# CSB5/lofreq

Hardware: AMD Instinct MI355X
Metric: pileup columns/sec at depth 10000 (higher is better)
Workload: dtype f64

## Files before the change

### lofreq_amd/csrc/lfq_api.hip

```cpp
#include "lfq_bound.h"
#include "lfq_ctx.h"

namespace {

struct LfqDeviceStreams {
    hipStream_t stream = nullptr, dps = nullptr, side[2] = {nullptr, nullptr};
    hipEvent_t ev_tail[3] = {nullptr, nullptr, nullptr};
    bool tail_recorded = false;
    hipEvent_t ev_end = nullptr;
    bool end_recorded = false;
    int refs = 0;
};
std::mutex g_streams_m;
LfqDeviceStreams g_streams[64];

bool acquire_streams(int device, lfq_ctx *c);
void release_streams(int device);

void *pin_acquire_impl(lfq_ctx *c, size_t bytes, int *slot)
{
    int best = -1, empty = -1, smallest = -1;
    for (int i = 0; i < LFQ_PIN_SLOTS; i++) {
        auto &b = c->pin_pool[i];
        if (b.used) {
// ... 231 lines not shown
    for (;;) {
        {
            std::unique_lock<std::mutex> lk(*c->lm);
            c->lcv->wait(lk, [&] { return c->leader_go > 0 || c->leader_stop; });
            if (c->leader_stop) {
                return;
            }
            c->leader_go--;
        }
        int64_t n = 0;
        if (hipEventSynchronize(c->ev_heavy) == hipSuccess) {
            n = std::min<int64_t>(std::max<int64_t>(*(volatile int32_t *)c->h_nheavy, 0), c->heavy_cap);
        }
        lfq_sb_precompute(c->h_tuples, 3 * n);
        {
            std::lock_guard<std::mutex> lk(*c->lm);
            c->sb_pending--;
        }
        c->lcv->notify_all();
    }
}

int ensure_workspace(lfq_ctx *c, int64_t ncols)
{
    if (ncols > c->ws_cols) {
        int64_t cap = 0;
        int64_t want = ncols + ncols / 8 + 1024;
        if (c->d_flags) (void)hipFree(c->d_flags);
        if (c->d_prefix) (void)hipFree(c->d_prefix);
        if (c->d_entries) (void)hipFree(c->d_entries);
        if (c->d_tiles) (void)hipFree(c->d_tiles);
        if (c->d_unsplit) (void)hipFree(c->d_unsplit);
        if (c->d_retry) (void)hipFree(c->d_retry);
        c->d_unsplit = nullptr;
        c->d_retry = nullptr;
        c->d_flags = nullptr;
        c->d_prefix = nullptr;
        c->d_entries = nullptr;
        c->d_tiles = nullptr;
        c->ws_cols = 0;
        LFQ_TRY(grow(&c->d_flags, &cap, want));
        cap = 0;
        LFQ_TRY(grow(&c->d_prefix, &cap, want));
        cap = 0;
        LFQ_TRY(grow(&c->d_entries, &cap, want));
        cap = 0;
        LFQ_TRY(grow(&c->d_tiles, &cap, 2 * (want / 1024 + 8 * (LFQ_MAX_SEGMENTS + 1))));
        cap = 0;
        LFQ_TRY(grow(&c->d_unsplit, &cap, want));
        cap = 0;
        LFQ_TRY(grow(&c->d_retry, &cap, want));
        c->ws_cols = want;
    }
    return LFQ_OK;
}


}

void *lfq_pin_acquire(lfq_ctx *c, size_t bytes, int *slot) { return pin_acquire_impl(c, bytes, slot); }

extern "C" {

void *lfq_host_alloc(size_t bytes)
{
    void *p = nullptr;
    if (hipHostMalloc(&p, bytes ? bytes : 1, hipHostMallocDefault) != hipSuccess) {
        (void)hipGetLastError();
        return nullptr;
    }
    return p;
}

void lfq_host_free(void *p)
{
    if (p) {
        (void)hipHostFree(p);
    }
}
int lfq_create(lfq_ctx **out, int device_ordinal)
{
    if (!out) {
        return LFQ_ERR_INVALID;
    }
// ... 108 lines not shown
        if (c->h_pin2) (void)hipHostFree(c->h_pin2);
        if (c->d_detlim) (void)hipFree(c->d_detlim);
        if (c->d_sites_in) (void)hipFree(c->d_sites_in);
        if (c->d_sites_out) (void)hipFree(c->d_sites_out);
        for (int i = 0; i < 4; i++) {
            if (c->ev_sites_t[i]) (void)hipEventDestroy(c->ev_sites_t[i]);
        }
        if (c->d_sum) (void)hipFree(c->d_sum);
        if (c->h_sum) (void)hipHostFree(c->h_sum);
        delete c->plp_sum;
        if (c->ev_sum_t[0]) (void)hipEventDestroy(c->ev_sum_t[0]);
        if (c->ev_sum_t[1]) (void)hipEventDestroy(c->ev_sum_t[1]);
        if (c->ev_baq_t[0]) (void)hipEventDestroy(c->ev_baq_t[0]);
        if (c->ev_baq_t[1]) (void)hipEventDestroy(c->ev_baq_t[1]);
        if (c->ev_idq_t[0]) (void)hipEventDestroy(c->ev_idq_t[0]);
        if (c->ev_idq_t[1]) (void)hipEventDestroy(c->ev_idq_t[1]);
        if (c->d_baq_scr) (void)hipFree(c->d_baq_scr);
        if (c->d_baq_expect) (void)hipFree(c->d_baq_expect);
        if (c->d_baq_tmp8) (void)hipFree(c->d_baq_tmp8);
        if (c->d_baq_nflag) (void)hipFree(c->d_baq_nflag);
        if (c->d_baq_itab) (void)hipFree(c->d_baq_itab);
        if (c->d_baq_terms) (void)hipFree(c->d_baq_terms);
        lfq_viterbi_release(c);
        if (c->h_tuples) (void)hipHostFree(c->h_tuples);
        if (c->h_nheavy) (void)hipHostFree(c->h_nheavy);
        if (c->ev_heavy) (void)hipEventDestroy(c->ev_heavy);
    }
    if (!c) {
        return;
    }
    (void)hipSetDevice(c->device);
    if (c->stream) (void)hipStreamSynchronize(c->stream);
    void *bufs[] = {c->d_luts, c->d_flags, c->d_prefix, c->d_entries, c->d_counters, c->d_tiles, c->d_longs, c->d_pool, c->d_unsplit, c->d_retry,
                    c->d_scratch, c->d_counts, c->d_pvals, c->d_stage, c->d_approx_mu};
    for (void *b : bufs) {
        if (b) (void)hipFree(b);
    }
    if (c->h_counters) (void)hipHostFree(c->h_counters);
    for (int i = 0; i < 4; i++) {
        if (c->ev[i]) (void)hipEventDestroy(c->ev[i]);
    }
    for (int i = 0; i < 3; i++) {
        if (c->ev_join[i]) (void)hipEventDestroy(c->ev_join[i]);
        if (i == 0 && c->ev_segw) (void)hipEventDestroy(c->ev_segw);
        if (i == 0 && c->ev_prep) (void)hipEventDestroy(c->ev_prep);
        if (i == 0 && c->ev_mid) (void)hipEventDestroy(c->ev_mid);
    }
    for (int s = 0; s < LFQ_MAX_SEGMENTS; s++) {
        hipEvent_t evs[] = {c->ev_cnt[s][0], c->ev_cnt[s][1], c->ev_scan[s], c->ev_light[s][0], c->ev_light[s][1],
                            c->ev_side[0][s][0], c->ev_side[0][s][1], c->ev_side[1][s][0], c->ev_side[1][s][1]};
        for (hipEvent_t e : evs) {
            if (e) (void)hipEventDestroy(e);
        }
    }
    if (c->own_streams) {
        release_streams(c->device);
    }
    free(c);
}

int lfq_synchronize(lfq_ctx *c)
{
    if (!c) {
        return LFQ_ERR_INVALID;
    }
    LFQ_TRY_HIP(hipStreamSynchronize(c->stream));
    LFQ_TRY_HIP(hipEventSynchronize(c->ev[3]));
// ... 77 lines not shown
    }
    c->cur_col_bytes = 8 + 1 + (T.coverage_plp ? 4 : 0) + (T.num_bases ? 4 : 0) + (P.detlim_af ? 4 : 0);
    LFQ_TRY(lfq_order_after_batch(c, st));
    LFQ_TRY(tail_wait(c, st));
    LFQ_TRY_HIP(hipMemsetAsync(c->d_counters, 0, (LFQ_MAX_SEGMENTS + 1) * LFQ_NCOUNTERS * sizeof(int32_t), st));
    if (ncols > 0) {
        LFQ_TRY_HIP(hipMemsetAsync(c->d_retry, 0, (size_t)ncols, st));
    }
    LFQ_TRY_HIP(hipEventRecord(c->ev[0], st));
    if (ncols == 0) {
        LFQ_TRY_HIP(hipMemcpyAsync(c->h_counters, c->d_counters,
                                   (LFQ_MAX_SEGMENTS + 1) * LFQ_NCOUNTERS * sizeof(int32_t), hipMemcpyDeviceToHost, st));
        LFQ_TRY_HIP(hipEventRecord(c->ev[3], st));
        c->batch_recorded = 1;
        return LFQ_OK;
    }

    int64_t max_depth = tr->max_col_obs;
    if (max_depth <= 0) {
        LFQ_TRY(lfq_launch_maxdepth(T, gcounters, st));
        LFQ_TRY_HIP(hipMemcpyAsync(c->h_counters, gcounters, LFQ_NCOUNTERS * sizeof(int32_t), hipMemcpyDeviceToHost, st));
        LFQ_TRY_HIP(hipStreamSynchronize(st));
        max_depth = c->h_counters[LFQ_GC_MAXDEPTH];
    }
    {
        static const LfqLuts h_luts = [] {
            LfqLuts h;
            fill_luts(&h);
            return h;
        }();
        const bool lb = !P.general && P.def_alt_bq == 0 && P.def_alt_jp < 0.0;
        P.bound_p_lo = (lb && !indel_mode && kn.bound_gate && lfq_count_is_lean(T, P, max_depth))
                           ? lfq_bound_p_lo(h_luts.bq, P.min_alt_bq4, LFQ_BOUND_QLO) : 0.0;
    }
    const int64_t per_block = 3 * max_depth + 72;
    int n_big_blocks = c->n_cu;
    const int64_t budget = (int64_t)1 << 29;
    if (per_block * n_big_blocks > budget) {
        n_big_blocks = (int)std::max<int64_t>(8, budget / per_block);
    }
    LFQ_TRY(grow(&c->d_scratch, &c->scratch_doubles, per_block * n_big_blocks));
    if (!c->d_longs) {
        c->long_cap = 1 << 16;
        c->pool_cells = kn.split_pool_cells;
        LFQ_TRY_HIP(hipMalloc((void **)&c->d_longs, (size_t)c->long_cap * sizeof(LfqLong)));
        LFQ_TRY_HIP(hipMalloc((void **)&c->d_pool, (size_t)std::max(c->pool_cells, 1) * sizeof(LfqSegCell)));
        LFQ_TRY_HIP(hipEventCreateWithFlags(&c->ev_segw, hipEventDisableTiming));
        LFQ_TRY_HIP(hipEventCreateWithFlags(&c->ev_prep, hipEventDisableTiming));
        LFQ_TRY_HIP(hipEventCreateWithFlags(&c->ev_mid, hipEventDisableTiming));
    }

    const int n_seg = 1;
    c->cur_segments = n_seg;
    LFQ_TRY_HIP(hipEventRecord(c->ev_join[2], st));
    LFQ_TRY_HIP(hipStreamWaitEvent(dps, c->ev_join[2], 0));

    bool big_joined = false;
    for (int s = 0; s < n_seg; s++) {
        const int64_t c0 = ncols * s / n_seg, c1 = ncols * (s + 1) / n_seg;
        LfqWork W;
        W.tested_prefix = c->d_prefix;
        W.entries = c->d_entries + c0;
        W.counters = c->d_counters + s * LFQ_NCOUNTERS;
        W.gcounters = gcounters;
        W.block_sums = (int32_t *)(c->d_tiles + 2 * (c0 / 1024 + 8 * s));
        W.long_cap = c->long_cap / n_seg;
        W.pool_cells = c->pool_cells / n_seg;
        W.longs = c->d_longs + (int64_t)s * W.long_cap;
        W.pool = c->d_pool + (int64_t)s * W.pool_cells;
        W.unsplit = c->d_unsplit + c0;

        LFQ_TRY_HIP(hipEventRecord(c->ev_cnt[s][0], st));
        const bool ungated = c->batch_gate == LFQ_GATE_NONE && st == c->stream && !c->priv_stream_on && !single_stream;
        LFQ_TRY(lfq_launch_count(T, c0, c1, P, c->d_luts, d_counts, c->d_flags, max_depth, st, ungated));
        c->cur_sparse_counts = P.sparse_counts && lfq_count_is_shallow(T, P, max_depth);
        LFQ_TRY_HIP(hipEventRecord(c->ev_cnt[s][1], st));

        LFQ_TRY_HIP(hipStreamWaitEvent(dps, c->ev_cnt[s][1], 0));
        LFQ_TRY(lfq_launch_scan(T, c0, c1, c->d_flags, d_counts, W, dps));
        if (P.approx_n > 0) {
            LFQ_TRY(grow(&c->d_approx_mu, &c->approx_mu_bytes, (c1 - c0) * 8));
            LFQ_TRY(lfq_launch_approx_gate(T, P, c->d_luts, d_counts, W, c1 - c0, (double *)c->d_approx_mu, c->d_flags, dps));
            LFQ_TRY(lfq_launch_scan(T, c0, c1, c->d_flags, d_counts, W, dps, true));
        }
        LFQ_TRY_HIP(hipEventRecord(c->ev_scan[s], dps));
        const bool sb_heavy = n_seg == 1 && !indel_mode && c->leader && !kn.no_sb_precompute;
        auto launch_heavy = [&]() -> int {
            if (P.lazy_strand) {
                LFQ_TRY(lfq_launch_strand_heavy(T, W, d_counts, c->d_tuples_mapped, c->d_nheavy_mapped, c->heavy_cap, 16, dps));
            } else {
                LFQ_TRY(lfq_launch_gather_heavy(W, d_counts, c->d_tuples_mapped, c->d_nheavy_mapped, c->heavy_cap, 16, dps));
            }
            LFQ_TRY_HIP(hipEventRecord(c->ev_heavy, dps));
            {
                std::lock_guard<std::mutex> lk(*c->lm);
                c->leader_go++;
                c->sb_pending++;
            }
            c->lcv->notify_all();
            return LFQ_OK;
        };
        const bool screen = !kn.skip_light && kn.light_kernel != 2;
        if (sb_heavy && !screen) {
            LFQ_TRY(launch_heavy());
        }
        const int64_t seg_cols = c1 - c0;
        const int screen_auto = (c->batch_gate == LFQ_GATE_NONE && !indel_mode) ? (tr->max_col_obs >= 4096 ? 1 : 2) : 4;
        const int light_waves_per_cu = kn.light_kernel == 0 ? screen_auto : 10;
        const int n_light_waves = (int)std::min<int64_t>((int64_t)c->n_cu * light_waves_per_cu, std::max<int64_t>(seg_cols / 8, 4));
        const int n_mid_waves = (int)std::min<int64_t>((int64_t)c->n_cu * 4, std::max<int64_t>(seg_cols, 4));
        const bool run_big = !kn.skip_big, run_mid = !kn.skip_mid;
        const bool dbg_sync = kn.debug_sync != 0;
// ... 832 lines not shown
```

### lofreq_amd/csrc/lfq_ctx.h

```cpp
#ifndef LFQ_CTX_H
#define LFQ_CTX_H

#include <hip/hip_runtime.h>

#include <ctype.h>
#include <float.h>
#include <math.h>
#include <stdio.h>
#include <stdlib.h>
#include <string.h>

#include <algorithm>
#include <chrono>
#include <condition_variable>
#include <mutex>
#include <string>
#include <atomic>
#include <functional>
#include <unistd.h>
#include <fcntl.h>
#include <sys/file.h>
#include <thread>
#include <vector>

// ... 210 lines not shown
    std::vector<char> key_chars;
};

#define LFQ_PIN_SLOTS 40

struct lfq_ctx {
    int device;
    hipStream_t stream;
    LfqLuts *d_luts;
    int64_t ws_cols;
    uint8_t *d_flags;
    uint8_t *d_approx_mu;
    int64_t approx_mu_bytes;
    int32_t *d_prefix, *d_counters;
    LfqEntry *d_entries;
    hipStream_t dps;
    hipStream_t side[2];
    hipEvent_t ev_mid;
    hipEvent_t ev_cnt[LFQ_MAX_SEGMENTS][2];
    hipEvent_t ev_scan[LFQ_MAX_SEGMENTS];
    hipEvent_t ev_light[LFQ_MAX_SEGMENTS][2];
    hipEvent_t ev_side[2][LFQ_MAX_SEGMENTS][2];
    hipEvent_t ev_join[3];
    int cur_segments;
    uint64_t *d_tiles;
    double *d_scratch;
    int64_t scratch_doubles;
    LfqLong *d_longs;
    LfqSegCell *d_pool;
    int32_t long_cap, pool_cells;
    hipEvent_t ev_segw, ev_prep;
    int32_t *d_unsplit;
    uint8_t *d_retry;
    int32_t *h_counters;
    lfq_col_counts *d_counts;
    int64_t counts_cap;
    lfq_col_pvals *d_pvals;
    int64_t pvals_cap;
    uint8_t *d_stage;
    int64_t stage_bytes;
    hipStream_t cur_stream;
    int64_t cur_pvals_cap;
    int64_t cur_ncols;
    hipEvent_t ev[4];
    lfq_kernel_times times;
    lfq_dp_work work;
    int64_t cur_count_read, cur_count_written;
    const uint64_t *cur_col_off;
    int cur_obs_bytes_x2, cur_col_bytes;
    int cur_sparse_counts;
    int n_cu;
    int32_t *h_tuples, *d_tuples_mapped;
    int32_t *h_nheavy, *d_nheavy_mapped;
    int heavy_cap;
    hipEvent_t ev_heavy;
    uint8_t *d_plp_in, *d_plp_out;
    int64_t plp_in_bytes, plp_out_bytes;
    uint8_t *d_tmp[5];
    struct { void *p; size_t cap; } rs_cache[7];
    int priv_stream_on;
    hipStream_t priv_stream;
    hipStream_t up_stream;
    hipEvent_t ev_up;
    hipEvent_t ev_apply;
    uint8_t *h_pin;
    int64_t pin_bytes;
// ... 145 lines not shown
```

### lofreq_amd/csrc/lfq_dp.hip

```cpp
#include <atomic>

#include "lfq_bound.h"
#include "lfq_device.h"

#define LFQ_LN2_HI 6.93147180369123816490e-01
#define LFQ_LN2_LO 1.90821492927058770002e-10
#define LFQ_EXP_UNDERFLOW_X (-708.3964185322641)
#define LFQ_DBL_EPS 2.220446049250313e-16

#ifndef LFQ_HEAVY_WAVES
#define LFQ_HEAVY_WAVES 8
#endif
#ifndef LFQ_DP512_WAVES
#define LFQ_DP512_WAVES 2
#endif

struct LfqColCtx {
    int col;
    uint64_t off0;
    int64_t n_obs;
    int ref_code;
    int median_ref_bq;
    int K;
    int64_t bonf;
// ... 914 lines not shown
            pf.raw = nullptr;
            pf.entry = nullptr;
            lfq_wave_column<1, true, false>(cx, raw, T, P, &s_luts, rows, counts, W, pvals, pvals_capacity, pf);
        }
    }
}


template <int KREG>
__device__ __forceinline__ void lfq_screen_row(double (&v)[KREG], double p, double q)
{
    v[KREG - 1] = fma(v[KREG - 2], p, v[KREG - 1]);
#pragma unroll
    for (int j = KREG - 2; j >= 1; j--) {
        v[j] = fma(v[j - 1], p, v[j] * q);
    }
    v[0] = v[0] * q;
}

#define LFQ_SCREEN_BYTE(w4, j) \
    (((((j) >> 2) == 0 ? (w4).x : ((j) >> 2) == 1 ? (w4).y : ((j) >> 2) == 2 ? (w4).z : (w4).w) >> (8 * ((j) & 3))) & 0xffu)

#define LFQ_SCREEN_CLAIM 128

template <int KREG, bool LB, bool GATE>
__global__ __launch_bounds__(256) void lfq_dp_screen_kernel(LfqTracksDev T, LfqParams P,
                                                            const LfqLuts *__restrict__ g_luts, LfqWork W,
                                                            uint8_t *__restrict__ retry, int max_rounds)
{
    constexpr int MAXK = KREG - 1;
    static_assert(MAXK <= LFQ_BOUND_MAXK, "the bound gate's table");
    static_assert(LB || !GATE, "the bound needs the LB conditions");
    __shared__ LfqLuts s_luts;
    __shared__ LfqBoundTab s_bound;
    lfq_luts_to_lds(&s_luts, g_luts);
    if constexpr (GATE) {
        if (threadIdx.x < LFQ_BOUND_CODES) {
            s_bound.qm[threadIdx.x] = lfq_bound_qm(P.bound_p_lo, threadIdx.x);
        } else if (threadIdx.x >= 64 && threadIdx.x < 64 + LFQ_BOUND_NRK) {
            s_bound.rk[threadIdx.x - 64] = lfq_bound_rk(P.bound_p_lo, (int)threadIdx.x - 64);
        }
    }
    __syncthreads();
    const int lane = lfq_lane();
    const int n_work = W.counters[LFQ_CNT_LIGHT];
    const LfqEntry *list = W.entries;
    const double sig_s = P.sig * (1.0 + P.prune_slack);
    const LfqEvalMasks EM = lfq_eval_masks(P);
    const int xcd0 = (int)(blockIdx.x & 7u);
    int xcd_try = 0;
    int q_next = 0, q_end = 0;

    bool active = false;
    uint64_t off0 = 0;
    int n_obs = 0, rel = 0, K = 0, ref_code = 0, med = 0, rounds = 0, list_idx = 0, n_kept = 0;
    double bonf_d = 1.0;
    double v[KREG];
#pragma unroll
    for (int j = 0; j < KREG; j++) {
        v[j] = 0.0;
    }
    unsigned long long acc_cells = 0, acc_rows = 0;
    int n_retry = 0;

    for (;;) {
        uint64_t need = __ballot(!active);
        while (need != 0ull && (q_next < q_end || xcd_try < 8)) {
            if (q_next >= q_end) {
                const int x = (xcd0 + xcd_try) & 7;
                const int lo = (int)((int64_t)n_work * x / 8), hi = (int)((int64_t)n_work * (x + 1) / 8);
                int32_t *head = &W.counters[LFQ_CNT_XHEAD + 32 * x];
                int b = __hip_atomic_load(head, __ATOMIC_RELAXED, __HIP_MEMORY_SCOPE_AGENT);
                if (b < hi - lo) {
                    b = lfq_claim(head, LFQ_SCREEN_CLAIM);
                }
                if (b >= hi - lo) {
                    xcd_try++;
                    continue;
                }
                q_next = lo + b;
                q_end = min(lo + b + LFQ_SCREEN_CLAIM, hi);
            }
            const int idx = q_next + __popcll(need & ((1ull << lane) - 1ull));
            q_next = min(q_next + __popcll(need), q_end);
            if (!active && idx < q_end) {
                const uint4 *ep = reinterpret_cast<const uint4 *>(list + idx);
                const uint4 a = ep[0], b = ep[1];
                K = (int)b.y;
                if (K > MAXK) {
                    retry[idx] = 1;
                    n_retry++;
                } else {
                    int64_t bonf = P.bonf_base;
                    if (P.bonf_dynamic) {
                        bonf = ((P.bonf_reset_first && P.bonf_base == 1) ? 0 : P.bonf_base)
                               + (int64_t)P.bonf_step * (int)b.x;
                    }
                    bonf_d = (double)bonf;
                    active = true;
                    if constexpr (GATE) {
                        active = !(b.w != 0u && lfq_bound_tail(&s_bound, b.w & (LFQ_BOUND_CODES - 1u), K) * bonf_d > sig_s);
                    }
                    off0 = ((uint64_t)a.y << 32) | a.x;
                    n_obs = (int)a.z;
                    med = (int)(int16_t)(b.z & 0xffffu);
                    ref_code = (int)((b.z >> 16) & 0xffu);
                    rel = -(int)(off0 & 15u);
                    rounds = 0;
                    n_kept = 0;
                    list_idx = idx;
#pragma unroll
                    for (int j = 0; j < KREG; j++) {
                        v[j] = (j == MAXK - K) ? 1.0 : 0.0;
                    }
                }
            }
            need = __ballot(!active);
        }
        if (__ballot(active) == 0ull) {
            break;
        }

        uint4 bqw = make_uint4(0, 0, 0, 0), baqw = make_uint4(~0u, ~0u, ~0u, ~0u), mqw = make_uint4(0, 0, 0, 0);
        uint4 sqw = make_uint4(~0u, ~0u, ~0u, ~0u), ntw = make_uint4(0, 0, 0, 0);
        if (active) {
            const uint64_t wbase = (uint64_t)((int64_t)off0 + rel);
            bqw = *reinterpret_cast<const uint4 *>(T.bq + wbase);
            mqw = *reinterpret_cast<const uint4 *>(T.mq + wbase);
            if (!LB && T.baq) {
                baqw = *reinterpret_cast<const uint4 *>(T.baq + wbase);
            }
            if (!LB && T.sq) {
                sqw = *reinterpret_cast<const uint4 *>(T.sq + wbase);
            }
            if (T.nt_packed) {
// ... 1518 lines not shown
    }
    {
        static std::atomic<unsigned long long> allowed{0ull};
        int dev = 0;
        if (hipGetDevice(&dev) != hipSuccess) {
            return LFQ_ERR_HIP;
        }
        const unsigned long long bit = 1ull << (dev & 63);
        if (!(allowed.load(std::memory_order_acquire) & bit)) {
            const int bytes = (int)sizeof(LfqCombShared);
            if (hipFuncSetAttribute(reinterpret_cast<const void *>(&lfq_dp_combine_kernel<0>),
                                    hipFuncAttributeMaxDynamicSharedMemorySize, bytes) != hipSuccess ||
                hipFuncSetAttribute(reinterpret_cast<const void *>(&lfq_dp_combine_kernel<1>),
                                    hipFuncAttributeMaxDynamicSharedMemorySize, bytes) != hipSuccess) {
                return LFQ_ERR_HIP;
            }
            allowed.fetch_or(bit, std::memory_order_release);
        }
    }
    if (mode == 0) {
        hipLaunchKernelGGL(lfq_dp_fold_kernel<0>, dim3((unsigned)n_blocks * 4), dim3(64 * LFQ_FOLD_WAVES), 0,
                           (hipStream_t)stream, p, d_counts, w, d_pvals, pvals_capacity);
        hipLaunchKernelGGL(lfq_dp_combine_kernel<0>, dim3((unsigned)n_blocks), dim3(LFQ_COMB_THREADS), sizeof(LfqCombShared),
                           (hipStream_t)stream, p, d_counts, w, d_pvals, pvals_capacity, 1);
    } else {
        hipLaunchKernelGGL(lfq_dp_fold_kernel<1>, dim3((unsigned)n_blocks), dim3(64 * LFQ_FOLD_WAVES), 0,
                           (hipStream_t)stream, p, d_counts, w, d_pvals, pvals_capacity);
        hipLaunchKernelGGL(lfq_dp_combine_kernel<1>, dim3((unsigned)n_blocks), dim3(LFQ_COMB_THREADS), sizeof(LfqCombShared),
                           (hipStream_t)stream, p, d_counts, w, d_pvals, pvals_capacity, 1);
    }
    return hipGetLastError() == hipSuccess ? LFQ_OK : LFQ_ERR_HIP;
}

int lfq_launch_dp_quad(const LfqTracksDev &t, const LfqParams &p, const LfqLuts *d_luts,
                       const lfq_col_counts *d_counts, const LfqWork &w, uint8_t *d_retry, lfq_col_pvals *d_pvals,
                       int64_t pvals_capacity, int n_waves, int kreg_hint, void *stream, int phase)
{
    if (t.ncols <= 0 || n_waves <= 0) {
        return LFQ_OK;
    }
    const dim3 grid((unsigned)((n_waves + 3) / 4)), block(256);
    hipStream_t st = (hipStream_t)stream;
    const LfqKnobs &kn = lfq_knobs();
    int force = 0;
    if (phase != 2) {
        if (!force) {
            force = kreg_hint > 0 ? kreg_hint : 8;
        }
        const bool lb = !p.general && p.def_alt_bq == 0 && p.def_alt_jp < 0.0;
#define LFQ_LAUNCH_SCREEN(KR)                                                                                        \
    do {                                                                                                             \
        if (lb && p.bound_p_lo > 0.0) {                                                                              \
            hipLaunchKernelGGL((lfq_dp_screen_kernel<KR, true, true>), grid, block, 0, st, t, p, d_luts, w, d_retry, \
                               kn.screen_rounds);                                                                    \
        } else if (lb) {                                                                                             \
            hipLaunchKernelGGL((lfq_dp_screen_kernel<KR, true, false>), grid, block, 0, st, t, p, d_luts, w, d_retry, \
                               kn.screen_rounds);                                                                    \
        } else {                                                                                                     \
            hipLaunchKernelGGL((lfq_dp_screen_kernel<KR, false, false>), grid, block, 0, st, t, p, d_luts, w, d_retry, \
                               kn.screen_rounds);                                                                    \
        }                                                                                                            \
    } while (0)
        if (force <= 6) LFQ_LAUNCH_SCREEN(6);
        else if (force <= 8) LFQ_LAUNCH_SCREEN(8);
        else if (force <= 10) LFQ_LAUNCH_SCREEN(10);
        else if (force <= 12) LFQ_LAUNCH_SCREEN(12);
        else if (force <= 16) LFQ_LAUNCH_SCREEN(16);
        else if (force <= 24) LFQ_LAUNCH_SCREEN(24);
        else if (force <= 32) LFQ_LAUNCH_SCREEN(32);
        else {
            hipLaunchKernelGGL(lfq_dp_wave_kernel<1>, grid, block, 0, st, t, p, d_luts, d_counts, w, -1, LFQ_CNT_LIGHT,
                               d_pvals, pvals_capacity, 32, 0);
        }
#undef LFQ_LAUNCH_SCREEN
    }
    if (phase != 1) {
        hipLaunchKernelGGL(lfq_dp_retry_kernel, grid, block, 0, st, t, p, d_luts, d_counts, w, d_retry, d_pvals,
                           pvals_capacity);
    }
    return hipGetLastError() == hipSuccess ? LFQ_OK : LFQ_ERR_HIP;
}
```

### lofreq_amd/csrc/lfq_internal.h

```cpp
#ifndef LFQ_INTERNAL_H
#define LFQ_INTERNAL_H

#include <stdint.h>

#include "lofreq_amd.h"

struct LfqLuts {
    double bq[256];
    double baq[256];
    double mq[256];
    double sq[256];
};

struct LfqParams {
    int32_t min_bq4;
    int32_t min_alt_bq4;
    int32_t def_alt_bq;
    int32_t general;
    double jq_reject_above;
    double alt_jq_reject_above;
    double def_alt_jp;
    int32_t min_cov;
    int32_t use_baq, use_mq, use_sq;
    int32_t bonf_dynamic;
// ... 65 lines not shown
    int64_t pad_[4];
};

#define LFQ_SEG_MAX 8
#define LFQ_SEG_CLASSES 5
#define LFQ_SEG_MIN_CHUNKS 16
#ifndef LFQ_SEG_MIN_CHUNKS_SHORT
#define LFQ_SEG_MIN_CHUNKS_SHORT 4
#endif
#define LFQ_SEG_SHORT_BELOW 48
#define LFQ_PHASE1_CHUNKS 8
#define LFQ_SEG_BUDGET 4096
#define LFQ_SPLIT_MAX_K 2016

#if defined(__HIPCC__)
__host__ __device__
#endif
static inline int lfq_khist_thr(int f)
{
    return f == 0 ? 5 : f == 1 ? 7 : f == 2 ? 9 : f == 3 ? 11 : f == 4 ? 15 : f == 5 ? 23 : 31;
}

struct LfqWork {
    int32_t *tested_prefix;
    LfqEntry *entries;
    int32_t *gcounters;
    int32_t *counters;
    int32_t *block_sums;
    LfqLong *longs;
    int32_t *unsplit;
    LfqSegCell *pool;
    int32_t long_cap;
    int32_t pool_cells;
};

#define LFQ_MID_K 64
#define LFQ_BIG_K 250
#define LFQ_NCOUNTERS 320
#define LFQ_MAX_SEGMENTS 1
#define LFQ_GC_PVALS 0
#define LFQ_GC_OVERFLOW 1
#define LFQ_GC_TESTED 2
#define LFQ_GC_MAXDEPTH 3
#define LFQ_GC_CELLS 8
#define LFQ_GC_ROWS 10
#define LFQ_GC_APPROX_PRUNED 13
#define LFQ_GC_SCREEN_RETRY 12
#define LFQ_CNT_TESTED 0
#define LFQ_CNT_BIG 1
#define LFQ_CNT_MID 2
#define LFQ_CNT_LIGHT 3
#define LFQ_CNT_HEAD 4
#define LFQ_CNT_CARRY_IN 15
#define LFQ_CNT_HEAD_LIGHT 12
#define LFQ_CNT_HEAD_MID 13
#define LFQ_CNT_UNSPLIT 5
#define LFQ_CNT_HEAD_PREP 6
#define LFQ_CNT_POOL 7
#define LFQ_CNT_HEAD_COMB 24
#define LFQ_CNT_HEAD_FOLD 48
#define LFQ_CNT_KLE7 26
#define LFQ_CNT_KLE15 27
#define LFQ_CNT_KLE31 28
#define LFQ_CNT_XHEAD 64
#define LFQ_CNT_KHIST 40
#define LFQ_NKHIST 7
#define LFQ_CNT_LONG0 16

#define LFQ_SEQ_LETTERS "ACGTN=MRSVWYHKDB"
#if defined(__HIPCC__)
__host__ __device__
#endif
static inline char lfq_seq_letter(unsigned code)
{
    return code > 15u ? 'N' : LFQ_SEQ_LETTERS[code];
}

struct LfqKnobs {
    int timing;
    int single_stream;
    int no_sb_precompute;
    int debug_sync;
    int skip_light, skip_mid, skip_big;
    int light_kernel;
    int screen_rounds;
    int seg_max;
    int seg_max_mid;
    int split_pool_cells;
    long count_multi_below;
    int big_on_side;
    int baq_one_variant;
    int pileup_tiles;
    long host_loop_threads;
    long count_lpg4_below, count_lpg8_below;
    long host_spin_us;
    int sync_upload;
    int host_threads;
// ... 189 lines not shown
#define LFQ_SRCQ_PERFECT 1
#define LFQ_SRCQ_VALUE 2
struct LfqSrcqArgs {
    int64_t n_reads;
    const int32_t *pos;
    const int64_t *cigar_off, *seq_off;
    const uint32_t *cigar;
    const uint8_t *seq, *qual;
    const char *ref;
    int64_t ref_len;
    const uint8_t *ign;
    int32_t nonmatch_qual, min_bq;
    double *scratch;
    int64_t scratch_cells;
    double *prob;
    uint8_t *status;
};
int lfq_launch_srcq(const LfqSrcqArgs &a, const LfqLuts *d_luts, int n_blocks, void *stream);
int lfq_launch_pileup_scatter(const LfqPileupArgs &a, void *stream);

int lfq_launch_strand_heavy(const LfqTracksDev &t, const LfqWork &w, lfq_col_counts *d_counts, int32_t *tuples_mapped,
                            int32_t *n_mapped, int cap_entries, int min_alt, void *stream);
int lfq_launch_strand_pvals(const LfqTracksDev &t, lfq_col_pvals *d_pvals, const int32_t *d_n_pvals, int64_t cap, int n_blocks,
                            void *stream);
int lfq_launch_gather_heavy(const LfqWork &w, const lfq_col_counts *d_counts, int32_t *tuples_mapped,
                            int32_t *n_mapped, int cap_entries, int min_alt, void *stream);
int lfq_launch_maxdepth(const LfqTracksDev &t, int32_t *d_gcounters, void *stream);
int lfq_launch_ntcount(const LfqTracksDev &t, int32_t *d_out, void *stream);
bool lfq_count_is_shallow(const LfqTracksDev &t, const LfqParams &p, int64_t max_col_obs);
int lfq_launch_count(const LfqTracksDev &t, int64_t c0, int64_t c1, const LfqParams &p, const LfqLuts *d_luts,
                     lfq_col_counts *d_counts, uint8_t *d_flags, int64_t max_col_obs, void *stream, bool shallow_half_cu = false);
bool lfq_count_is_lean(const LfqTracksDev &t, const LfqParams &p, int64_t max_col_obs);
int lfq_launch_scan(const LfqTracksDev &t, int64_t c0, int64_t c1, const uint8_t *d_flags,
                    const lfq_col_counts *d_counts, const LfqWork &w, void *stream, bool relist = false);
int lfq_launch_approx_gate(const LfqTracksDev &t, const LfqParams &p, const LfqLuts *d_luts, const lfq_col_counts *d_counts,
                           const LfqWork &w, int64_t ncols_seg, double *d_mu, uint8_t *d_flags, void *stream);
int lfq_launch_dp_light(const LfqTracksDev &t, const LfqParams &p, const LfqLuts *d_luts,
                        const lfq_col_counts *d_counts, const LfqWork &w, lfq_col_pvals *d_pvals,
                        int64_t pvals_capacity, int n_waves, void *stream);
int lfq_launch_dp_quad(const LfqTracksDev &t, const LfqParams &p, const LfqLuts *d_luts,
                       const lfq_col_counts *d_counts, const LfqWork &w, uint8_t *d_retry, lfq_col_pvals *d_pvals,
                       int64_t pvals_capacity, int n_waves, int kreg_hint, void *stream, int phase = 0);
int lfq_launch_dp_mid(const LfqTracksDev &t, const LfqParams &p, const LfqLuts *d_luts,
                      const lfq_col_counts *d_counts, const LfqWork &w, lfq_col_pvals *d_pvals,
                      int64_t pvals_capacity, int n_waves, void *stream);
int lfq_launch_dp_big(const LfqTracksDev &t, const LfqParams &p, const LfqLuts *d_luts,
                      const lfq_col_counts *d_counts, const LfqWork &w, lfq_col_pvals *d_pvals,
                      int64_t pvals_capacity, double *d_scratch, int64_t scratch_doubles_per_block,
                      int n_blocks, void *stream);
int lfq_launch_dp_big_prep(const LfqTracksDev &t, const LfqParams &p, const LfqLuts *d_luts,
                           const lfq_col_counts *d_counts, const LfqWork &w, lfq_col_pvals *d_pvals,
                           int64_t pvals_capacity, int n_blocks, void *stream);
int lfq_launch_dp_seg(int mode, const LfqTracksDev &t, const LfqParams &p, const LfqLuts *d_luts,
                      const LfqWork &w, int n_waves, void *stream);
int lfq_launch_dp_combine(int mode, const LfqParams &p, const lfq_col_counts *d_counts, const LfqWork &w,
                          lfq_col_pvals *d_pvals, int64_t pvals_capacity, int n_blocks, void *stream);
int lfq_launch_synth(const struct lfq_synth_spec *d_spec_host, int64_t col_begin, int64_t ncols,
                     uint8_t *d_nt, uint8_t *d_bq, uint8_t *d_baq, uint8_t *d_mq, uint64_t *d_col_off,
                     uint8_t *d_ref_base, int nt_packed, void *stream);

#endif
```

### lofreq_amd/csrc/lfq_kernels.hip

```cpp
#include <hip/hip_runtime.h>
#include <math.h>
#include <stdint.h>

#include <algorithm>

#include "lfq_bound.h"
#include "lfq_device.h"
#include "lofreq_synth.h"


__device__ __forceinline__ uint32_t lfq_bytes_mask(int lo, int hi, int d)
{
    int l = lo - 4 * d, h = hi - 4 * d;
    l = l < 0 ? 0 : (l > 4 ? 4 : l);
    h = h < 0 ? 0 : (h > 4 ? 4 : h);
    const uint32_t below_h = (h >= 4) ? 0xFFFFFFFFu : ((1u << (8 * h)) - 1u);
    const uint32_t below_l = (l >= 4) ? 0xFFFFFFFFu : ((1u << (8 * l)) - 1u);
    return below_h & ~below_l & 0x80808080u;
}

struct LfqAcc {
    uint32_t raw[4], fw[4], ge[4], ga[4];
};

// ... 1273 lines not shown
        LfqTriple total;
        LfqTriple ex = lfq_block_excl_scan(x, &total, s_wave);
        if (i < ntiles) {
            lfq_triple_add(ex, carry);
            tile_sums[i] = ex;
        }
        lfq_triple_add(carry, total);
    }
    if (RELIST) {
        if (threadIdx.x == 0) {
            counters[LFQ_CNT_MID] = (int32_t)carry.m;
            counters[LFQ_CNT_BIG] = (int32_t)carry.b;
            counters[LFQ_CNT_LIGHT] = (int32_t)(carry.t - carry.m - carry.b);
        }
        if (threadIdx.x < 3) {
            counters[LFQ_CNT_KLE7 + (int)threadIdx.x] = 0;
        }
        if (threadIdx.x < LFQ_NKHIST) {
            counters[LFQ_CNT_KHIST + (int)threadIdx.x] = 0;
        }
        return;
    }
    if (threadIdx.x == 0) {
        counters[LFQ_CNT_TESTED] = (int32_t)carry.t;
        counters[LFQ_CNT_MID] = (int32_t)carry.m;
        counters[LFQ_CNT_BIG] = (int32_t)carry.b;
        counters[LFQ_CNT_LIGHT] = (int32_t)(carry.t - carry.m - carry.b);
        const int32_t before = gcounters[LFQ_GC_TESTED];
        counters[LFQ_CNT_CARRY_IN] = before;
        gcounters[LFQ_GC_TESTED] = before + (int32_t)carry.t;
    }
}

template <bool RELIST>
__global__ __launch_bounds__(LFQ_SCAN_THREADS) void lfq_scan_apply_kernel(LfqTracksDev T, int64_t c0, int64_t c1,
                                                                         const uint8_t *__restrict__ flags,
                                                                         const lfq_col_counts *__restrict__ counts,
                                                                         const LfqTriple *__restrict__ tile_sums,
                                                                         LfqWork W)
{
    __shared__ LfqTriple s_wave[16];
    const int64_t ncols = c1;
    const int64_t base = c0 + (int64_t)blockIdx.x * LFQ_SCAN_TILE + (int64_t)threadIdx.x * LFQ_SCAN_ITEMS;
    uint32_t f[LFQ_SCAN_ITEMS];
    LfqTriple x = {0, 0, 0};
    for (int i = 0; i < LFQ_SCAN_ITEMS; i++) {
        f[i] = (base + i < ncols) ? flags[base + i] : 0u;
        lfq_triple_add(x, lfq_triple_of_flag(f[i]));
    }
    LfqTriple total;
    LfqTriple ex = lfq_block_excl_scan(x, &total, s_wave);
    lfq_triple_add(ex, tile_sums[blockIdx.x]);
    const uint32_t base_mid = (uint32_t)W.counters[LFQ_CNT_LIGHT];
    const uint32_t base_big = base_mid + (uint32_t)W.counters[LFQ_CNT_MID];
    const uint32_t carry_in = (uint32_t)W.counters[LFQ_CNT_CARRY_IN];
    uint32_t kle7 = 0, kle15 = 0, kle31 = 0;
    unsigned long long khist = 0;
    for (int i = 0; i < LFQ_SCAN_ITEMS; i++) {
        const int64_t c = base + i;
        if (c >= ncols) {
            break;
        }
        if (f[i] & 1u) {
            uint32_t pos;
            const lfq_col_counts *cn = &counts[c];
            if (f[i] & 4u) {
                pos = base_big + ex.b++;
            } else if (f[i] & 2u) {
                pos = base_mid + ex.m++;
            } else {
                pos = ex.t - ex.m - ex.b;
                kle7 += cn->kmax <= 7;
                kle15 += cn->kmax <= 15;
                kle31 += cn->kmax <= 31;
#pragma unroll
                for (int f = 0; f < LFQ_NKHIST; f++) {
                    khist += (unsigned long long)(cn->kmax <= lfq_khist_thr(f)) << (9 * f);
                }
            }
            ex.t++;
            const uint32_t rb = T.ref_base[c];
            LfqEntry e;
            e.off0 = T.col_off[c];
            e.n_obs = (int32_t)(T.col_off[c + 1] - e.off0);
            e.col = (int32_t)c;
            e.prefix = RELIST ? W.tested_prefix[c] : (int32_t)(carry_in + ex.t);
            e.kmax = cn->kmax;
            e.median_ref_bq = (int16_t)cn->median_ref_bq;
            e.ref_code = (uint8_t)((rb == 'A') ? 0 : (rb == 'C') ? 1 : (rb == 'G') ? 2 : 3);
            e.pad_ = 0;
            e.pad2_ = (f[i] & 6u) ? 0 : (int32_t)(f[i] >> LFQ_FLAG_NLO_SHIFT);
            W.entries[pos] = e;
        }
        if (!RELIST) {
            W.tested_prefix[c] = (int32_t)(carry_in + ex.t);
        }
    }
    __shared__ uint32_t s_k[3 + LFQ_NKHIST];
    if (threadIdx.x < 3 + LFQ_NKHIST) {
        s_k[threadIdx.x] = 0;
    }
    __syncthreads();
    kle7 = lfq_wave_sum_u32(kle7);
    kle15 = lfq_wave_sum_u32(kle15);
    kle31 = lfq_wave_sum_u32(kle31);
#pragma unroll
    for (int d = 32; d >= 1; d >>= 1) {
        khist += __shfl_xor(khist, d, 64);
    }
    if (lfq_lane() == 0 && kle31) {
        atomicAdd(&s_k[0], kle7);
        atomicAdd(&s_k[1], kle15);
        atomicAdd(&s_k[2], kle31);
#pragma unroll
        for (int f = 0; f < LFQ_NKHIST; f++) {
            atomicAdd(&s_k[3 + f], (uint32_t)((khist >> (9 * f)) & 511ull));
        }
    }
    __syncthreads();
    if (threadIdx.x < 3 && s_k[2]) {
        atomicAdd(&W.counters[LFQ_CNT_KLE7 + (int)threadIdx.x], (int)s_k[threadIdx.x]);
    }
    if (threadIdx.x >= 3 && threadIdx.x < 3 + LFQ_NKHIST && s_k[2]) {
        atomicAdd(&W.counters[LFQ_CNT_KHIST + (int)threadIdx.x - 3], (int)s_k[threadIdx.x]);
    }
}


__global__ __launch_bounds__(256) void lfq_synth_kernel(lfq_synth_spec S, int64_t col_begin, int64_t ncols,
                                                        uint8_t *__restrict__ nt, uint8_t *__restrict__ bq,
                                                        uint8_t *__restrict__ baq, uint8_t *__restrict__ mq,
                                                        uint64_t *__restrict__ col_off,
                                                        uint8_t *__restrict__ ref_base, int nt_packed)
{
    const int64_t total = ncols * (int64_t)S.depth;
    const int64_t n16 = (total + 15) / 16;
    const int64_t stride = (int64_t)gridDim.x * blockDim.x;
    for (int64_t t = (int64_t)blockIdx.x * blockDim.x + threadIdx.x; t < n16; t += stride) {
        uint32_t wn[4] = {0, 0, 0, 0}, wb[4] = {0, 0, 0, 0}, wa[4] = {0, 0, 0, 0}, wm[4] = {0, 0, 0, 0};
        for (int b = 0; b < 16; b++) {
            const int64_t g = t * 16 + b;
            lfq_synth_obs o;
            if (g < total) {
                const int64_t c = g / S.depth;
                o = lfq_synth_observation(&S, (uint64_t)(col_begin + c), (uint64_t)(g - c * S.depth));
            } else {
                o.nt = 4;
                o.bq = 0;
                o.baq = 0;
                o.mq = 0;
            }
            wn[b >> 2] |= (uint32_t)o.nt << (8 * (b & 3));
            wb[b >> 2] |= (uint32_t)o.bq << (8 * (b & 3));
            wa[b >> 2] |= (uint32_t)o.baq << (8 * (b & 3));
            wm[b >> 2] |= (uint32_t)o.mq << (8 * (b & 3));
        }
        if (nt_packed) {
// ... 134 lines not shown
            else hipLaunchKernelGGL((lfq_count_lean_kernel<false>), dim3(blocks), wg, 0, (hipStream_t)stream, ca, d_counts, d_flags, c0, c1);
            LFQ_HIP_TRY(hipGetLastError());
            return LFQ_OK;
        }
#define LFQ_LAUNCH_F(PK, ST, SM)                                                                                     \
    hipLaunchKernelGGL((lfq_count_fast_kernel<PK, ST, SM>), dim3(blocks), wg, 0, (hipStream_t)stream, ca, d_counts, d_flags, c0, c1)
        switch (variant) {
        case 0: LFQ_LAUNCH_F(false, false, false); break;
        case 1: LFQ_LAUNCH_F(false, false, true); break;
        case 2: LFQ_LAUNCH_F(false, true, false); break;
        case 3: LFQ_LAUNCH_F(false, true, true); break;
        case 6: LFQ_LAUNCH_F(true, true, false); break;
        default: LFQ_LAUNCH_F(true, true, true); break;
        }
#undef LFQ_LAUNCH_F
        LFQ_HIP_TRY(hipGetLastError());
        return LFQ_OK;
    }
    const unsigned blocks = (unsigned)((c1 - c0 + 3) / 4);
#define LFQ_LAUNCH_COUNT(PK, ST)                                                                                     \
    hipLaunchKernelGGL((lfq_count_kernel<PK, ST>), dim3(blocks), dim3(256), 0, (hipStream_t)stream, t, p, d_luts,       \
                       d_counts, d_flags, c0, c1)
    if (t.nt_packed) {
        if (strand) LFQ_LAUNCH_COUNT(true, true); else LFQ_LAUNCH_COUNT(true, false);
    } else {
        if (strand) LFQ_LAUNCH_COUNT(false, true); else LFQ_LAUNCH_COUNT(false, false);
    }
#undef LFQ_LAUNCH_COUNT
    LFQ_HIP_TRY(hipGetLastError());
    return LFQ_OK;
}

int lfq_launch_scan(const LfqTracksDev &t, int64_t c0, int64_t c1, const uint8_t *d_flags,
                    const lfq_col_counts *d_counts, const LfqWork &w, void *stream, bool relist)
{
    const int64_t ncols = c1 - c0;
    if (ncols <= 0) {
        return LFQ_OK;
    }
    const int64_t ntiles = (ncols + LFQ_SCAN_TILE - 1) / LFQ_SCAN_TILE;
    LfqTriple *tile_sums = reinterpret_cast<LfqTriple *>(w.block_sums);
    hipLaunchKernelGGL(lfq_scan_tiles_kernel, dim3((unsigned)ntiles), dim3(LFQ_SCAN_THREADS), 0,
                       (hipStream_t)stream, ncols, d_flags + c0, tile_sums);
    if (relist) {
        hipLaunchKernelGGL(lfq_scan_sums_kernel<true>, dim3(1), dim3(LFQ_SCAN_THREADS), 0, (hipStream_t)stream, ntiles,
                           tile_sums, w.counters, w.gcounters);
        hipLaunchKernelGGL(lfq_scan_apply_kernel<true>, dim3((unsigned)ntiles), dim3(LFQ_SCAN_THREADS), 0,
                           (hipStream_t)stream, t, c0, c1, d_flags, d_counts, (const LfqTriple *)tile_sums, w);
    } else {
        hipLaunchKernelGGL(lfq_scan_sums_kernel<false>, dim3(1), dim3(LFQ_SCAN_THREADS), 0, (hipStream_t)stream, ntiles,
                           tile_sums, w.counters, w.gcounters);
        hipLaunchKernelGGL(lfq_scan_apply_kernel<false>, dim3((unsigned)ntiles), dim3(LFQ_SCAN_THREADS), 0,
                           (hipStream_t)stream, t, c0, c1, d_flags, d_counts, (const LfqTriple *)tile_sums, w);
    }
    LFQ_HIP_TRY(hipGetLastError());
    return LFQ_OK;
}

int lfq_launch_synth(const lfq_synth_spec *spec, int64_t col_begin, int64_t ncols, uint8_t *d_nt,
                     uint8_t *d_bq, uint8_t *d_baq, uint8_t *d_mq, uint64_t *d_col_off, uint8_t *d_ref_base,
                     int nt_packed, void *stream)
{
    if (ncols <= 0) {
        return LFQ_OK;
    }
    const int64_t n16 = (ncols * (int64_t)spec->depth + 15) / 16;
    int64_t blocks = (n16 + 255) / 256;
    if (blocks > 256 * 32) {
        blocks = 256 * 32;
    }
    if (blocks < 1) {
        blocks = 1;
    }
    hipLaunchKernelGGL(lfq_synth_kernel, dim3((unsigned)blocks), dim3(256), 0, (hipStream_t)stream, *spec,
                       col_begin, ncols, d_nt, d_bq, d_baq, d_mq, d_col_off, d_ref_base, nt_packed);
    LFQ_HIP_TRY(hipGetLastError());
    return LFQ_OK;
}


template <bool PACKED>
__device__ __forceinline__ void lfq_strand_of_column(const LfqTracksDev &T, int64_t col, int *ref_fw, int *ref_rv,
                                                     int alt_fw[3], int alt_raw[3])
{
    const uint64_t off0 = T.col_off[col], off1 = T.col_off[col + 1];
    LfqAcc a;
// ... 153 lines not shown
```

Before: 360.9 million.

## Move bound-gate screening into scan apply and emit compact survivor list

The Poisson bound gate used to be evaluated inside the DP screen kernel, where every light entry was loaded and then possibly discarded. It now runs in the scan-apply kernel, which writes a compacted list of surviving entry indices plus a survivor count. The screen kernel iterates only over those survivors through an extra indirection, which cuts wasted lanes and per-block bound-table setup. The cost is a new workspace buffer, extra atomics and a serial per-thread write loop in the scan, plus gate parameters and the kreg selection duplicated on the host side.

```diff
diff --git a/lofreq_amd/csrc/lfq_api.hip b/lofreq_amd/csrc/lfq_api.hip
--- a/lofreq_amd/csrc/lfq_api.hip
+++ b/lofreq_amd/csrc/lfq_api.hip
@@ -287,8 +287,10 @@
         if (c->d_tiles) (void)hipFree(c->d_tiles);
         if (c->d_unsplit) (void)hipFree(c->d_unsplit);
         if (c->d_retry) (void)hipFree(c->d_retry);
+        if (c->d_surv) (void)hipFree(c->d_surv);
         c->d_unsplit = nullptr;
         c->d_retry = nullptr;
+        c->d_surv = nullptr;
         c->d_flags = nullptr;
         c->d_prefix = nullptr;
         c->d_entries = nullptr;
@@ -305,6 +307,8 @@
         LFQ_TRY(grow(&c->d_unsplit, &cap, want));
         cap = 0;
         LFQ_TRY(grow(&c->d_retry, &cap, want));
+        cap = 0;
+        LFQ_TRY(grow(&c->d_surv, &cap, want));
         c->ws_cols = want;
     }
     return LFQ_OK;
@@ -479,7 +483,7 @@
     (void)hipSetDevice(c->device);
     if (c->stream) (void)hipStreamSynchronize(c->stream);
     void *bufs[] = {c->d_luts, c->d_flags, c->d_prefix, c->d_entries, c->d_counters, c->d_tiles, c->d_longs, c->d_pool, c->d_unsplit, c->d_retry,
-                    c->d_scratch, c->d_counts, c->d_pvals, c->d_stage, c->d_approx_mu};
+                    c->d_surv, c->d_scratch, c->d_counts, c->d_pvals, c->d_stage, c->d_approx_mu};
     for (void *b : bufs) {
         if (b) (void)hipFree(b);
     }
@@ -623,6 +627,10 @@
         const bool lb = !P.general && P.def_alt_bq == 0 && P.def_alt_jp < 0.0;
         P.bound_p_lo = (lb && !indel_mode && kn.bound_gate && lfq_count_is_lean(T, P, max_depth))
                            ? lfq_bound_p_lo(h_luts.bq, P.min_alt_bq4, LFQ_BOUND_QLO) : 0.0;
+    }
+    const int screen_kreg = lfq_screen_kreg(indel_mode ? c->kreg_hint_indel : c->kreg_hint);
+    if (kn.skip_light || kn.light_kernel == 2 || screen_kreg == 0 || P.approx_n > 0) {
+        P.bound_p_lo = 0.0;
     }
     const int64_t per_block = 3 * max_depth + 72;
     int n_big_blocks = c->n_cu;
@@ -660,6 +668,7 @@
         W.longs = c->d_longs + (int64_t)s * W.long_cap;
         W.pool = c->d_pool + (int64_t)s * W.pool_cells;
         W.unsplit = c->d_unsplit + c0;
+        W.surv = c->d_surv + c0;
 
         LFQ_TRY_HIP(hipEventRecord(c->ev_cnt[s][0], st));
         const bool ungated = c->batch_gate == LFQ_GATE_NONE && st == c->stream && !c->priv_stream_on && !single_stream;
@@ -668,7 +677,17 @@
         LFQ_TRY_HIP(hipEventRecord(c->ev_cnt[s][1], st));
 
         LFQ_TRY_HIP(hipStreamWaitEvent(dps, c->ev_cnt[s][1], 0));
-        LFQ_TRY(lfq_launch_scan(T, c0, c1, c->d_flags, d_counts, W, dps));
+        {
+            LfqScanGate G;
+            G.p_lo = P.bound_p_lo;
+            G.sig_s = P.sig * (1.0 + P.prune_slack);
+            G.bonf_base = P.bonf_base;
+            G.bonf_dynamic = P.bonf_dynamic;
+            G.bonf_step = P.bonf_step;
+            G.bonf_reset_first = P.bonf_reset_first;
+            G.maxk = screen_kreg - 1;
+            LFQ_TRY(lfq_launch_scan(T, c0, c1, c->d_flags, d_counts, W, dps, false, P.bound_p_lo > 0.0 ? &G : nullptr));
+        }
         if (P.approx_n > 0) {
             LFQ_TRY(grow(&c->d_approx_mu, &c->approx_mu_bytes, (c1 - c0) * 8));
             LFQ_TRY(lfq_launch_approx_gate(T, P, c->d_luts, d_counts, W, c1 - c0, (double *)c->d_approx_mu, c->d_flags, dps));
diff --git a/lofreq_amd/csrc/lfq_ctx.h b/lofreq_amd/csrc/lfq_ctx.h
--- a/lofreq_amd/csrc/lfq_ctx.h
+++ b/lofreq_amd/csrc/lfq_ctx.h
@@ -266,6 +266,7 @@
     hipEvent_t ev_segw, ev_prep;
     int32_t *d_unsplit;
     uint8_t *d_retry;
+    int32_t *d_surv;
     int32_t *h_counters;
     lfq_col_counts *d_counts;
     int64_t counts_cap;
diff --git a/lofreq_amd/csrc/lfq_dp.hip b/lofreq_amd/csrc/lfq_dp.hip
--- a/lofreq_amd/csrc/lfq_dp.hip
+++ b/lofreq_amd/csrc/lfq_dp.hip
@@ -970,18 +970,10 @@
     static_assert(MAXK <= LFQ_BOUND_MAXK, "the bound gate's table");
     static_assert(LB || !GATE, "the bound needs the LB conditions");
     __shared__ LfqLuts s_luts;
-    __shared__ LfqBoundTab s_bound;
     lfq_luts_to_lds(&s_luts, g_luts);
-    if constexpr (GATE) {
-        if (threadIdx.x < LFQ_BOUND_CODES) {
-            s_bound.qm[threadIdx.x] = lfq_bound_qm(P.bound_p_lo, threadIdx.x);
-        } else if (threadIdx.x >= 64 && threadIdx.x < 64 + LFQ_BOUND_NRK) {
-            s_bound.rk[threadIdx.x - 64] = lfq_bound_rk(P.bound_p_lo, (int)threadIdx.x - 64);
-        }
-    }
     __syncthreads();
     const int lane = lfq_lane();
-    const int n_work = W.counters[LFQ_CNT_LIGHT];
+    const int n_work = W.counters[GATE ? LFQ_CNT_SURV : LFQ_CNT_LIGHT];
     const LfqEntry *list = W.entries;
     const double sig_s = P.sig * (1.0 + P.prune_slack);
     const LfqEvalMasks EM = lfq_eval_masks(P);
@@ -1019,9 +1011,10 @@
                 q_next = lo + b;
                 q_end = min(lo + b + LFQ_SCREEN_CLAIM, hi);
             }
-            const int idx = q_next + __popcll(need & ((1ull << lane) - 1ull));
+            const int slot = q_next + __popcll(need & ((1ull << lane) - 1ull));
             q_next = min(q_next + __popcll(need), q_end);
-            if (!active && idx < q_end) {
+            if (!active && slot < q_end) {
+                const int idx = GATE ? W.surv[slot] : slot;
                 const uint4 *ep = reinterpret_cast<const uint4 *>(list + idx);
                 const uint4 a = ep[0], b = ep[1];
                 K = (int)b.y;
@@ -1036,9 +1029,6 @@
                     }
                     bonf_d = (double)bonf;
                     active = true;
-                    if constexpr (GATE) {
-                        active = !(b.w != 0u && lfq_bound_tail(&s_bound, b.w & (LFQ_BOUND_CODES - 1u), K) * bonf_d > sig_s);
-                    }
                     off0 = ((uint64_t)a.y << 32) | a.x;
                     n_obs = (int)a.z;
                     med = (int)(int16_t)(b.z & 0xffffu);
@@ -2623,6 +2613,13 @@
     return hipGetLastError() == hipSuccess ? LFQ_OK : LFQ_ERR_HIP;
 }
 
+int lfq_screen_kreg(int kreg_hint)
+{
+    const int force = kreg_hint > 0 ? kreg_hint : 8;
+    return force <= 6 ? 6 : force <= 8 ? 8 : force <= 10 ? 10 : force <= 12 ? 12 : force <= 16 ? 16 : force <= 24 ? 24
+           : force <= 32 ? 32 : 0;
+}
+
 int lfq_launch_dp_quad(const LfqTracksDev &t, const LfqParams &p, const LfqLuts *d_luts,
                        const lfq_col_counts *d_counts, const LfqWork &w, uint8_t *d_retry, lfq_col_pvals *d_pvals,
                        int64_t pvals_capacity, int n_waves, int kreg_hint, void *stream, int phase)
@@ -2635,9 +2632,7 @@
     const LfqKnobs &kn = lfq_knobs();
     int force = 0;
     if (phase != 2) {
-        if (!force) {
-            force = kreg_hint > 0 ? kreg_hint : 8;
-        }
+        force = lfq_screen_kreg(kreg_hint);
         const bool lb = !p.general && p.def_alt_bq == 0 && p.def_alt_jp < 0.0;
 #define LFQ_LAUNCH_SCREEN(KR)                                                                                        \
     do {                                                                                                             \
@@ -2652,13 +2647,13 @@
                                kn.screen_rounds);                                                                    \
         }                                                                                                            \
     } while (0)
-        if (force <= 6) LFQ_LAUNCH_SCREEN(6);
-        else if (force <= 8) LFQ_LAUNCH_SCREEN(8);
-        else if (force <= 10) LFQ_LAUNCH_SCREEN(10);
-        else if (force <= 12) LFQ_LAUNCH_SCREEN(12);
-        else if (force <= 16) LFQ_LAUNCH_SCREEN(16);
-        else if (force <= 24) LFQ_LAUNCH_SCREEN(24);
-        else if (force <= 32) LFQ_LAUNCH_SCREEN(32);
+        if (force == 6) LFQ_LAUNCH_SCREEN(6);
+        else if (force == 8) LFQ_LAUNCH_SCREEN(8);
+        else if (force == 10) LFQ_LAUNCH_SCREEN(10);
+        else if (force == 12) LFQ_LAUNCH_SCREEN(12);
+        else if (force == 16) LFQ_LAUNCH_SCREEN(16);
+        else if (force == 24) LFQ_LAUNCH_SCREEN(24);
+        else if (force == 32) LFQ_LAUNCH_SCREEN(32);
         else {
             hipLaunchKernelGGL(lfq_dp_wave_kernel<1>, grid, block, 0, st, t, p, d_luts, d_counts, w, -1, LFQ_CNT_LIGHT,
                                d_pvals, pvals_capacity, 32, 0);
diff --git a/lofreq_amd/csrc/lfq_internal.h b/lofreq_amd/csrc/lfq_internal.h
--- a/lofreq_amd/csrc/lfq_internal.h
+++ b/lofreq_amd/csrc/lfq_internal.h
@@ -121,6 +121,15 @@
     LfqSegCell *pool;
     int32_t long_cap;
     int32_t pool_cells;
+    int32_t *surv;
+};
+
+struct LfqScanGate {
+    double p_lo;
+    double sig_s;
+    int64_t bonf_base;
+    int32_t bonf_dynamic, bonf_step, bonf_reset_first;
+    int32_t maxk;
 };
 
 #define LFQ_MID_K 64
@@ -152,6 +161,7 @@
 #define LFQ_CNT_KLE15 27
 #define LFQ_CNT_KLE31 28
 #define LFQ_CNT_XHEAD 64
+#define LFQ_CNT_SURV 56
 #define LFQ_CNT_KHIST 40
 #define LFQ_NKHIST 7
 #define LFQ_CNT_LONG0 16
@@ -407,7 +417,9 @@
                      lfq_col_counts *d_counts, uint8_t *d_flags, int64_t max_col_obs, void *stream, bool shallow_half_cu = false);
 bool lfq_count_is_lean(const LfqTracksDev &t, const LfqParams &p, int64_t max_col_obs);
 int lfq_launch_scan(const LfqTracksDev &t, int64_t c0, int64_t c1, const uint8_t *d_flags,
-                    const lfq_col_counts *d_counts, const LfqWork &w, void *stream, bool relist = false);
+                    const lfq_col_counts *d_counts, const LfqWork &w, void *stream, bool relist = false,
+                    const LfqScanGate *gate = nullptr);
+int lfq_screen_kreg(int kreg_hint);
 int lfq_launch_approx_gate(const LfqTracksDev &t, const LfqParams &p, const LfqLuts *d_luts, const lfq_col_counts *d_counts,
                            const LfqWork &w, int64_t ncols_seg, double *d_mu, uint8_t *d_flags, void *stream);
 int lfq_launch_dp_light(const LfqTracksDev &t, const LfqParams &p, const LfqLuts *d_luts,
diff --git a/lofreq_amd/csrc/lfq_kernels.hip b/lofreq_amd/csrc/lfq_kernels.hip
--- a/lofreq_amd/csrc/lfq_kernels.hip
+++ b/lofreq_amd/csrc/lfq_kernels.hip
@@ -1329,14 +1329,24 @@
     }
 }
 
-template <bool RELIST>
+template <bool RELIST, bool GATE = false>
 __global__ __launch_bounds__(LFQ_SCAN_THREADS) void lfq_scan_apply_kernel(LfqTracksDev T, int64_t c0, int64_t c1,
                                                                          const uint8_t *__restrict__ flags,
                                                                          const lfq_col_counts *__restrict__ counts,
                                                                          const LfqTriple *__restrict__ tile_sums,
-                                                                         LfqWork W)
-{
+                                                                         LfqWork W, LfqScanGate G)
+{
+    static_assert(!(RELIST && GATE), "the second pass of a batch with the Poisson gate has no bound gate");
     __shared__ LfqTriple s_wave[16];
+    __shared__ LfqBoundTab s_bound;
+    __shared__ uint32_t s_surv[2];
+    if constexpr (GATE) {
+        if (threadIdx.x < LFQ_BOUND_CODES) {
+            s_bound.qm[threadIdx.x] = lfq_bound_qm(G.p_lo, threadIdx.x);
+        } else if (threadIdx.x >= 64 && threadIdx.x < 64 + LFQ_BOUND_NRK) {
+            s_bound.rk[threadIdx.x - 64] = lfq_bound_rk(G.p_lo, (int)threadIdx.x - 64);
+        }
+    }
     const int64_t ncols = c1;
     const int64_t base = c0 + (int64_t)blockIdx.x * LFQ_SCAN_TILE + (int64_t)threadIdx.x * LFQ_SCAN_ITEMS;
     uint32_t f[LFQ_SCAN_ITEMS];
@@ -1353,6 +1363,7 @@
     const uint32_t carry_in = (uint32_t)W.counters[LFQ_CNT_CARRY_IN];
     uint32_t kle7 = 0, kle15 = 0, kle31 = 0;
     unsigned long long khist = 0;
+    uint32_t light0 = 0, n_mine = 0, surv_mask = 0;
     for (int i = 0; i < LFQ_SCAN_ITEMS; i++) {
         const int64_t c = base + i;
         if (c >= ncols) {
@@ -1388,6 +1399,26 @@
             e.pad_ = 0;
             e.pad2_ = (f[i] & 6u) ? 0 : (int32_t)(f[i] >> LFQ_FLAG_NLO_SHIFT);
             W.entries[pos] = e;
+            if constexpr (GATE) {
+                if (!(f[i] & 6u)) {
+                    const uint32_t code = (uint32_t)e.pad2_;
+                    bool gated = false;
+                    if (e.kmax <= G.maxk) {
+                        int64_t bonf = G.bonf_base;
+                        if (G.bonf_dynamic) {
+                            bonf = ((G.bonf_reset_first && G.bonf_base == 1) ? 0 : G.bonf_base)
+                                   + (int64_t)G.bonf_step * e.prefix;
+                        }
+                        gated = code != 0u
+                                && lfq_bound_tail(&s_bound, code & (LFQ_BOUND_CODES - 1u), e.kmax) * (double)bonf > G.sig_s;
+                    }
+                    if (n_mine == 0) {
+                        light0 = pos;
+                    }
+                    surv_mask |= (gated ? 0u : 1u) << n_mine;
+                    n_mine++;
+                }
+            }
         }
         if (!RELIST) {
             W.tested_prefix[c] = (int32_t)(carry_in + ex.t);
@@ -1397,7 +1428,16 @@
     if (threadIdx.x < 3 + LFQ_NKHIST) {
         s_k[threadIdx.x] = 0;
     }
+    if (GATE && threadIdx.x == 0) {
+        s_surv[0] = 0;
+    }
     __syncthreads();
+    uint32_t surv_rank = 0;
+    if constexpr (GATE) {
+        if (surv_mask) {
+            surv_rank = atomicAdd(&s_surv[0], (uint32_t)__popc(surv_mask));
+        }
+    }
     kle7 = lfq_wave_sum_u32(kle7);
     kle15 = lfq_wave_sum_u32(kle15);
     kle31 = lfq_wave_sum_u32(kle31);
@@ -1420,6 +1460,18 @@
     }
     if (threadIdx.x >= 3 && threadIdx.x < 3 + LFQ_NKHIST && s_k[2]) {
         atomicAdd(&W.counters[LFQ_CNT_KHIST + (int)threadIdx.x - 3], (int)s_k[threadIdx.x]);
+    }
+    if constexpr (GATE) {
+        if (threadIdx.x == 0 && s_surv[0]) {
+            s_surv[1] = (uint32_t)atomicAdd(&W.counters[LFQ_CNT_SURV], (int)s_surv[0]);
+        }
+        __syncthreads();
+        uint32_t at = s_surv[1] + surv_rank;
+        for (uint32_t j = 0; j < n_mine; j++) {
+            if ((surv_mask >> j) & 1u) {
+                W.surv[at++] = (int32_t)(light0 + j);
+            }
+        }
     }
 }
 
@@ -1620,7 +1672,7 @@
 }
 
 int lfq_launch_scan(const LfqTracksDev &t, int64_t c0, int64_t c1, const uint8_t *d_flags,
-                    const lfq_col_counts *d_counts, const LfqWork &w, void *stream, bool relist)
+                    const lfq_col_counts *d_counts, const LfqWork &w, void *stream, bool relist, const LfqScanGate *gate)
 {
     const int64_t ncols = c1 - c0;
     if (ncols <= 0) {
@@ -1634,12 +1686,17 @@
         hipLaunchKernelGGL(lfq_scan_sums_kernel<true>, dim3(1), dim3(LFQ_SCAN_THREADS), 0, (hipStream_t)stream, ntiles,
                            tile_sums, w.counters, w.gcounters);
         hipLaunchKernelGGL(lfq_scan_apply_kernel<true>, dim3((unsigned)ntiles), dim3(LFQ_SCAN_THREADS), 0,
-                           (hipStream_t)stream, t, c0, c1, d_flags, d_counts, (const LfqTriple *)tile_sums, w);
+                           (hipStream_t)stream, t, c0, c1, d_flags, d_counts, (const LfqTriple *)tile_sums, w, LfqScanGate{});
     } else {
         hipLaunchKernelGGL(lfq_scan_sums_kernel<false>, dim3(1), dim3(LFQ_SCAN_THREADS), 0, (hipStream_t)stream, ntiles,
                            tile_sums, w.counters, w.gcounters);
-        hipLaunchKernelGGL(lfq_scan_apply_kernel<false>, dim3((unsigned)ntiles), dim3(LFQ_SCAN_THREADS), 0,
-                           (hipStream_t)stream, t, c0, c1, d_flags, d_counts, (const LfqTriple *)tile_sums, w);
+        if (gate) {
+            hipLaunchKernelGGL((lfq_scan_apply_kernel<false, true>), dim3((unsigned)ntiles), dim3(LFQ_SCAN_THREADS), 0,
+                               (hipStream_t)stream, t, c0, c1, d_flags, d_counts, (const LfqTriple *)tile_sums, w, *gate);
+        } else {
+            hipLaunchKernelGGL(lfq_scan_apply_kernel<false>, dim3((unsigned)ntiles), dim3(LFQ_SCAN_THREADS), 0,
+                               (hipStream_t)stream, t, c0, c1, d_flags, d_counts, (const LfqTriple *)tile_sums, w, LfqScanGate{});
+        }
     }
     LFQ_HIP_TRY(hipGetLastError());
     return LFQ_OK;
diff --git a/profiles/count_gap.py b/profiles/count_gap.py
--- /dev/null
+++ b/profiles/count_gap.py
@@ -0,0 +1,28 @@
+#!/usr/bin/env python
+import glob
+import sqlite3
+import statistics
+import sys
+
+d = sys.argv[1]
+n_last = int(sys.argv[2]) if len(sys.argv) > 2 else 20
+db = d if d.endswith(".db") else sorted(glob.glob(d + "/**/*.db", recursive=True))[-1]
+con = sqlite3.connect(db)
+rows = con.execute("select name, start, end, grid_x, workgroup_x from kernels order by start").fetchall()
+idx = [i for i, r in enumerate(rows) if "lfq_count_" in r[0]]
+gaps, fills = [], []
+for a, b in zip(idx[:-1], idx[1:]):
+    gaps.append((rows[b][1] - rows[a][2]) / 1e3)
+    fills.append([(r[2] - r[1]) / 1e3 for r in rows[a + 1:b] if "fillBuffer" in r[0] and r[1] >= rows[a][2]])
+gaps, fills = gaps[-n_last:], fills[-n_last:]
+if gaps:
+    print("count end -> next count start, last %d pairs: median %.1f  min %.1f  max %.1f us" % (
+        len(gaps), statistics.median(gaps), min(gaps), max(gaps)))
+    print("  fills that start inside that gap: median count %d, median summed duration %.1f us" % (
+        statistics.median([len(f) for f in fills]), statistics.median([sum(f) for f in fills])))
+for key in ("lfq_dp_screen_kernel", "lfq_scan_apply_kernel", "lfq_count_"):
+    sel = [r for r in rows if key in r[0]][-n_last:]
+    if sel:
+        dur = [(r[2] - r[1]) / 1e3 for r in sel]
+        print("%-22s last %d: median %.1f  min %.1f  max %.1f us; grid %s x wg %s (%s)" % (
+            key, len(sel), statistics.median(dur), min(dur), max(dur), sel[-1][3], sel[-1][4], sel[-1][0][:60]))
```

Measured after the change: 356.1 million. 1.3% lower.
